# syl051088/DynaAlign

Hardware: AMD Instinct MI355X
Metric: sequence-pairs/sec (MinHash k=4 n_hash=500; NW BLOSUM62) at 1/2/4/8 MI355X (higher is better)
Workload: dtype u32

## Files before the change

dynaalign_amd/csrc/api.cpp:

```cpp
#include <sched.h>

#include <algorithm>
#include <atomic>
#include <chrono>
#include <climits>
#include <cmath>
#include <condition_variable>
#include <cstddef>
#include <map>
#include <memory>
#include <cstdlib>
#include <cstring>
#include <functional>
#include <mutex>
#include <random>
#include <string>
#include <thread>
#include <vector>

#include "da_common.hpp"

namespace da { size_t destroy_cached_comms(); }

namespace da {
// ... 345 lines not shown
  c.mh_no_pipe = env_flag("DYNAALIGN_MH_NO_PIPE");
  c.mh_pipe_one_stream = env_flag("DYNAALIGN_MH_PIPE_ONE_STREAM");
  c.mh_dedup_min_n = env_i64("DYNAALIGN_MH_DEDUP_MIN_N", -1);
  c.mh_dedup_max_pct = env_i64("DYNAALIGN_MH_DEDUP_MAX_PCT", -1);
  c.mh_sparse_max_pairs = std::min<uint64_t>(env_u64("DYNAALIGN_MH_SPARSE_MAX_PAIRS", 400000000ull), 0xfffffff0ull);
  c.mh_no_hybrid = env_flag("DYNAALIGN_MH_NO_HYBRID");
  c.mh_hybrid_min_n = env_i64("DYNAALIGN_MH_HYBRID_MIN_N", -1);
  c.mh_hybrid_dedup = env_flag("DYNAALIGN_MH_HYBRID_DEDUP");
  if (const char *e = getenv("DYNAALIGN_MH_EXPAND"))
    c.mh_expand = !strcmp(e, "rows") ? MH_EXPAND_ROWS : !strcmp(e, "rowspipe") ? MH_EXPAND_ROWSPIPE : !strcmp(e, "pipe") ? MH_EXPAND_PIPE
                : !strcmp(e, "tiles") ? MH_EXPAND_TILES : MH_EXPAND_DEFAULT;
  c.mh_pipe_step = (int)std::max<int64_t>(0, env_i64("DYNAALIGN_MH_PIPE_STEP", 0));
  c.mh_pipe_wg = (int)std::max<int64_t>(0, std::min<int64_t>(4, env_i64("DYNAALIGN_MH_PIPE_WG", 0)));
  c.mh_pipe_head = (int)std::max<int64_t>(0, env_i64("DYNAALIGN_MH_PIPE_HEAD", 0));
  c.mh_expand_zones = (int)env_i64("DYNAALIGN_MH_EXPAND_ZONES", 0);
  const int pb = (int)env_i64("DYNAALIGN_PLANE_BITS", 0);
  c.plane_bits = (pb == 32 || pb == 16 || pb == 15 || pb == 14 || pb == 12) ? pb : 0;
  c.k2_no_asm = env_flag("DYNAALIGN_K2_NO_ASM");
  c.k2_persist = env_flag("DYNAALIGN_K2_PERSIST");
  c.k2_wg_per_cu = (int)std::max<int64_t>(0, env_i64("DYNAALIGN_K2_WG_PER_CU", 0));
  c.nw_no_dedup = env_flag("DYNAALIGN_NW_NO_DEDUP");
  c.nw_int32 = env_flag("DYNAALIGN_NW_INT32");
  c.nw_no_prefix = env_flag("DYNAALIGN_NW_NO_PREFIX_SHARE");
  c.nw_dedup_min_n = env_i64("DYNAALIGN_NW_DEDUP_MIN_N", -1);
  c.no_host_widen = env_flag("DYNAALIGN_NO_HOST_WIDEN");
  c.plain_d2h = env_flag("DYNAALIGN_PLAIN_D2H");
  c.no_buffer_cache = env_flag("DYNAALIGN_NO_BUFFER_CACHE");
  c.d2h_threads = (int)std::max<int64_t>(0, env_i64("DYNAALIGN_D2H_THREADS", 0));
  c.buffer_cache_pct = (int)std::max<int64_t>(0, std::min<int64_t>(90, env_i64("DYNAALIGN_BUFFER_CACHE_PCT", 30)));
  c.block_bytes = env_u64("DYNAALIGN_BLOCK_BYTES", 0);
// ... 200 lines not shown
    (void)hipStreamSynchronize(r->side); (void)hipStreamSynchronize(r->alt[0]); (void)hipStreamSynchronize(r->alt[1]);
    std::lock_guard<std::mutex> g(pipe_pool().m);
    pipe_pool().idle[r->dev & 63].push_back(r);
  }
};
static int count_unique(const uint8_t *d_bytes, const int64_t *d_offsets, int64_t n, const NwDedupPlan &p, hipStream_t stream, int64_t *U) {
  int rc;
  if ((rc = launch_nw_dedup_count(d_bytes, d_offsets, n, p, stream)) != DA_OK) return rc;
  int32_t M = 0, S = 0;
  DA_HIP_TRY(hipMemcpyAsync(&M, p.pm + n, 4, hipMemcpyDeviceToHost, stream));
  DA_HIP_TRY(hipMemcpyAsync(&S, p.ps + n, 4, hipMemcpyDeviceToHost, stream));
  DA_HIP_TRY(hipStreamSynchronize(stream));
  *U = (int64_t)M + S; return DA_OK;
}
enum MhForm { MH_DIRECT = 0, MH_TILES = 1, MH_SPARSE = 2, MH_TILES_PIPE = 3, MH_ROWS = 4, MH_ROWS_PIPE = 5 };
struct MhRoute { int64_t n = 0, unique = 0, hybrid_pairs = -1; int taken = MH_DIRECT, plane_bits = 0, chunks = 0, expand_launches = 0, hybrid_bits_before = 0; bool packed_table = false; float ms[6] = {0, 0, 0, 0, 0, 0}; };
static MhRoute &mh_route() { static thread_local MhRoute r; return r; }
struct MhEvents {
  hipEvent_t e[7] = {nullptr, nullptr, nullptr, nullptr, nullptr, nullptr, nullptr};
  ~MhEvents() { for (hipEvent_t x : e) if (x) (void)hipEventDestroy(x); }
  hipEvent_t operator[](int i) const { return e[i]; }
  static void ms(MhRoute &r, int i, hipEvent_t from, hipEvent_t to) { (void)hipEventElapsedTime(&r.ms[i], from, to); }
  void steps(MhRoute &r, int count) const { for (int i = 0; i < count; ++i) ms(r, i, e[i], e[i + 1]); }
};
struct LaunchUnion {
  hipEvent_t origin; float total = 0, covered_to = 0;
  void add(hipEvent_t begin, hipEvent_t end) {
    float b = 0, e = 0;
    (void)hipEventElapsedTime(&b, origin, begin); (void)hipEventElapsedTime(&e, origin, end);
    if (e > covered_to) { total += e - std::max(b, covered_to); covered_to = e; }
  }
};
struct MhDedup { int64_t U = 0; bool take = false, rows = false; DevBuf work; NwDedupPlan p{}; std::vector<int32_t> ub; };
static int mh_count_unique(const uint8_t *d_res, const int64_t *d_off, int64_t n, int64_t total, DevBuf *work, NwDedupPlan *p, int64_t *U,
                           hipStream_t stream) {
  int rc;
  if ((rc = work->alloc(nw_dedup_workspace_bytes(n, total))) != DA_OK) return rc;
  *p = nw_dedup_layout(work->p, n, total);
  return count_unique(d_res, d_off, n, *p, stream, U);
}
static int mh_dedup_plan(const uint8_t *d_res, const int64_t *d_off, int64_t n, int64_t total, int n_hash, const double *d_out, int64_t ld,
                         MhDedup *d, hipStream_t stream) {
  const Config &cfg = da::config();
  int rc;
  d->U = n;
  const int64_t min_n = cfg.mh_dedup_min_n >= 0 ? cfg.mh_dedup_min_n : 2048;
  if (n < min_n || n > 0x7ffffff0LL || total <= 0 || n_hash > 2047 || cfg.mh_no_dedup) return DA_OK;
  if ((rc = mh_count_unique(d_res, d_off, n, total, &d->work, &d->p, &d->U, stream)) != DA_OK) return rc;
  const int64_t U = d->U;
  const int64_t max_pct = cfg.mh_dedup_max_pct >= 0 ? cfg.mh_dedup_max_pct
                        : expand_stream_ok(n, std::min<int64_t>(U, 65536), n_hash, d_out, ld) ? 68 : 60;
  d->take = U > 0 && U * 100 <= n * max_pct && expand_rows_workspace_bytes(n, U, DA_OUT_F64, false, n_hash, 0) != 0;
  if (!d->take) return DA_OK;
  if ((rc = launch_nw_dedup_build(d_res, d_off, n, U, d->p, stream, true)) != DA_OK) return rc;
  d->rows = cfg.mh_expand <= MH_EXPAND_ROWSPIPE && expand_stream_ok(n, U, n_hash, d_out, ld);
  if (d->rows) return DA_OK;
  const int64_t NB = mh_sym_bands(n);
  std::vector<int32_t> b((size_t)NB);
  d->ub.resize((size_t)NB + 1);
  DA_HIP_TRY(hipMemcpy2DAsync(d->ub.data(), 4, d->p.pm, 4096, 4, (size_t)NB, hipMemcpyDeviceToHost, stream));
  DA_HIP_TRY(hipMemcpy2DAsync(b.data(), 4, d->p.ps, 4096, 4, (size_t)NB, hipMemcpyDeviceToHost, stream));
  DA_HIP_TRY(hipStreamSynchronize(stream));
  for (int64_t q = 0; q < NB; ++q) d->ub[(size_t)q] += b[(size_t)q];
  d->ub[(size_t)NB] = (int32_t)U;
  return DA_OK;
}
constexpr int HY_KEEP = 254;
enum class MhOperand { dense, sparse, split };
struct MhAdmission { MhOperand form = MhOperand::dense; uint64_t pairs = 0; const uint16_t *codes = nullptr, *dense = nullptr; int64_t ld_ids = 0; };
static int mh_admit(const Dictionary &dict, void *d_work, int64_t n, int n_hash, bool ask_sparse, int split_from_bits, MhAdmission *a,
// ... 226 lines not shown
}
}

static int mh_full_symmetric(const uint8_t *d_res, const int64_t *d_off, int64_t n, int64_t total, int k, int n_hash,
                             const uint32_t *d_seeds, double *d_out, int64_t ld, hipStream_t stream) {
  const Config &cfg = da::config();
  int rc;
  MhRoute &route = mh_route() = MhRoute();
  route.n = n;
  MhEvents ev;
  for (auto &e : ev.e) DA_HIP_TRY(hipEventCreate(&e));
  DA_HIP_TRY(hipEventRecord(ev[0], stream));
  MhDedup d;
  if ((rc = mh_dedup_plan(d_res, d_off, n, total, n_hash, d_out, ld, &d, stream)) != DA_OK) return rc;
  route.unique = d.U;
  DA_HIP_TRY(hipEventRecord(ev[1], stream));
  MhCodes c;
  if ((rc = mh_codes(d.take ? d.p.ucodes : d_res, d.take ? d.p.uoff : d_off, d.take ? d.U : n, k, n_hash, d_seeds, !d.take && d.U * 10 >= n * 9,
                     d.take && !cfg.mh_hybrid_dedup ? 13 : 12, &c, stream)) != DA_OK) return rc;
  route.plane_bits = c.bits;
  if (c.split()) { route.hybrid_pairs = (int64_t)c.adm.pairs; route.hybrid_bits_before = c.dict.bits_data; }
  DA_HIP_TRY(hipEventRecord(ev[2], stream));
  MhCall call{n, n_hash, d_out, ld, stream, route, ev, c, d};
  if (!d.take) return c.adm.form == MhOperand::sparse ? mh_sparse(call) : mh_direct(call);
  DevBuf dtab, ex;
  call.pk = d.rows && !c.split() && mh_compare_pk_ok(d.U, n_hash, c.bits);
  route.packed_table = call.pk;
  call.ld_d = call.pk ? pk_lo_bytes(d.U) : (d.U + 7) / 8 * 8;
  if ((rc = dtab.alloc(call.pk ? pk_table_bytes(d.U) : (size_t)d.U * (size_t)call.ld_d * 2)) != DA_OK) return rc;
  if ((rc = ex.alloc(d.rows ? expand_stream_scratch_bytes(n, d.U) : expand_rows_workspace_bytes(n, d.U, DA_OUT_F64, false, n_hash, 0))) != DA_OK) return rc;
// ... 13 lines not shown
  if (n_hash > 65535) return fail(DA_ERR_UNSUPPORTED, "the compare kernel counts in 16 bits: n_hash <= 65535 (got %d); da_similarity_mh handles more", n_hash);
  return mh_full_symmetric(d_residues, d_offsets, n, total_residues, k, n_hash, d_seeds, d_out, ld, static_cast<hipStream_t>(stream));
}

int da_mh_last_route_chunks(int *chunks_out, int *expand_launches_out) {
  const MhRoute &r = mh_route();
  if (chunks_out) *chunks_out = r.chunks;
  if (expand_launches_out) *expand_launches_out = r.expand_launches;
  return DA_OK;
}

int da_mh_last_route_split(int64_t *rare_incidences_out, int *plane_bits_without_out) {
  const MhRoute &r = mh_route();
  if (rare_incidences_out) *rare_incidences_out = r.hybrid_pairs;
  if (plane_bits_without_out) *plane_bits_without_out = r.hybrid_bits_before;
  return DA_OK;
}

extern "C" int da_debug_mh_last_table_packed(int *packed_out) {
  if (!packed_out) return fail(DA_ERR_BAD_ARG, "NULL pointer");
  *packed_out = mh_route().packed_table ? 1 : 0;
  return DA_OK;
}

int da_mh_last_route(int64_t *n_out, int64_t *unique_out, int *dedup_taken_out, int *plane_bits_out, double *ms6_out) {
  const MhRoute &r = mh_route();
  if (n_out) *n_out = r.n;
  if (unique_out) *unique_out = r.unique;
  if (dedup_taken_out) *dedup_taken_out = r.taken;
  if (plane_bits_out) *plane_bits_out = r.plane_bits;
// ... 68 lines not shown
  MhCrossRoute &route = mh_cross_route() = MhCrossRoute();
  route.m = m; route.n = n; route.ux = m; route.uy = n;
  CrossEvents ev;
  for (auto &e : ev.e) DA_HIP_TRY(hipEventCreate(&e));
  DA_HIP_TRY(hipEventRecord(ev.e[0], stream));
  CrossSide sx, sy;
  bool take = false;
  const int64_t min_n = cfg.mh_dedup_min_n >= 0 ? cfg.mh_dedup_min_n : 2048;
  if (!cfg.mh_no_dedup && m + n >= min_n && x_total > 0 && y_total > 0 && n_hash <= 2047) {
    if ((rc = mh_count_unique(d_x_residues, d_x_offsets, m, x_total, &sx.work, &sx.p, &sx.U, stream)) != DA_OK ||
        (rc = mh_count_unique(d_y_residues, d_y_offsets, n, y_total, &sy.work, &sy.p, &sy.U, stream)) != DA_OK) return rc;
    route.ux = sx.U; route.uy = sy.U;
    const double pct = (double)(cfg.mh_dedup_max_pct >= 0 ? cfg.mh_dedup_max_pct : 68);
    take = sx.U > 0 && sy.U > 0 && (double)sx.U * (double)sy.U * 10000.0 <= (double)m * (double)n * pct * pct &&
           expand_stream_rect_ok(m, n, sx.U, sy.U, n_hash, d_out, ld);
    if (take && ((rc = launch_nw_dedup_build(d_x_residues, d_x_offsets, m, sx.U, sx.p, stream, true)) != DA_OK ||
                 (rc = launch_nw_dedup_build(d_y_residues, d_y_offsets, n, sy.U, sy.p, stream, true)) != DA_OK)) return rc;
  }
  DA_HIP_TRY(hipEventRecord(ev.e[1], stream));
  MhCrossOperand c;
  if ((rc = take ? mh_cross_operand(sx.p.ucodes, sx.p.uoff, sx.U, sy.p.ucodes, sy.p.uoff, sy.U, k, n_hash, d_seeds, &c, stream)
                 : mh_cross_operand(d_x_residues, d_x_offsets, m, d_y_residues, d_y_offsets, n, k, n_hash, d_seeds, &c, stream)) != DA_OK) return rc;
  route.plane_bits = c.bits;
  DA_HIP_TRY(hipEventRecord(ev.e[2], stream));
  DevBuf dtab, ex;
  if (!take) {
    if ((rc = mh_cross_compare(c, n_hash, 0, m, DA_OUT_F64, d_out, ld, stream)) != DA_OK) return rc;
    DA_HIP_TRY(hipEventRecord(ev.e[3], stream));
  } else {
    const int64_t ld_d = (sy.U + 7) / 8 * 8;
    if ((rc = dtab.alloc((size_t)sx.U * (size_t)ld_d * 2)) != DA_OK || (rc = ex.alloc(expand_stream_scratch_bytes(m, sx.U))) != DA_OK) return rc;
    if ((rc = mh_cross_compare(c, n_hash, 0, sx.U, DA_OUT_COMPACT, dtab.p, ld_d, stream)) != DA_OK) return rc;
// ... 2925 lines not shown
```

dynaalign_amd/csrc/da_common.hpp:

```cpp
#pragma once

#include <hip/hip_runtime.h>

#include <cstdarg>
#include <cstdint>
#include <cstdio>
#include <string>

#include "../../include/dynaalign.h"

namespace da {
struct Config {
  bool mh_no_dedup = false, mh_no_sparse = false, mh_no_pipe = false, mh_pipe_one_stream = false;
  int64_t mh_dedup_min_n = -1, mh_dedup_max_pct = -1;
  uint64_t mh_sparse_max_pairs = 400000000ull;
  bool mh_no_hybrid = false, mh_hybrid_dedup = false;
  int64_t mh_hybrid_min_n = -1;
  int mh_expand = 0;
  int mh_pipe_step = 0, mh_pipe_wg = 0, mh_pipe_head = 0;
  int mh_expand_zones = 0;
  int plane_bits = 0;
  bool k2_no_asm = false, k2_persist = false;
  int k2_wg_per_cu = 0;
  bool nw_no_dedup = false, nw_int32 = false, nw_no_prefix = false;
  int64_t nw_dedup_min_n = -1;
  bool no_host_widen = false, plain_d2h = false, no_buffer_cache = false;
  int d2h_threads = 0, buffer_cache_pct = 30;
  uint64_t block_bytes = 0;
  bool trace = false, louvain_debug = false;
  int louvain_threads = 0;
};
const Config &config();


std::string &last_error_ref();
// ... 61 lines not shown
__host__ __device__ inline int64_t pad16_base_words(int64_t n, int n_hash) { return 2 * plane_geom(n, n_hash, 16).copy_words; }
__host__ __device__ inline int64_t pad16_slot_word(int64_t n, int n_hash, int64_t row, int group) {
  const int64_t nst = (n_hash + 31) / 32;
  return (((row >> 7) * nst + group) * 128 + k2_slot((int)(row & 127))) * K2_PAD16_SLOT_WORDS;
}
inline int64_t mh_planes_words(int64_t n, int n_hash) {
  if (n <= 0 || n_hash <= 0) return 0;
  const int64_t raw = 2 * plane_geom(n, n_hash, 32).copy_words;
  const int64_t p16 = pad16_base_words(n, n_hash) + 2 * pad16_copy_words(n, n_hash);
  return raw > p16 ? raw : p16;
}

__host__ __device__ inline int64_t pk_lo_bytes(int64_t U) { return (U + 127) / 128 * 128; }
__host__ __device__ inline int64_t pk_row_bytes(int64_t lo_bytes) { return lo_bytes + lo_bytes / 8; }
inline size_t pk_table_bytes(int64_t U) { return (size_t)U * (size_t)pk_row_bytes(pk_lo_bytes(U)); }

int launch_minhash_signatures(const uint8_t *d_res, const int64_t *d_off, int64_t n,
                              int k, int n_hash, const uint32_t *d_seeds, uint32_t *d_sig,
                              int64_t ld_sig, hipStream_t stream);
int launch_mh_compare(const uint32_t *d_planes, int64_t n, int n_hash,
                      int64_t row_begin, int64_t row_end, bool symmetric, int kind,
                      void *d_out, int64_t ld, hipStream_t stream, int plane_bits = 32, int tile_stride = 1,
                      bool upper_only = false, int fold_q = 0, int64_t fold_w = 0);
int launch_mh_compare_rect(const uint32_t *d_planes, int64_t n, int n_hash, int64_t row_begin, int64_t row_end, int64_t col_begin, int64_t col_end,
                           int kind, void *d_out, int64_t ld, hipStream_t stream, int plane_bits);
int launch_fill_sig_rows(uint32_t *d_sig, int64_t ld_sig, int64_t m, int64_t m_pad, int n_hash, hipStream_t stream);
int64_t mh_sym_bands(int64_t n);
int64_t mh_sym_band_prefix(int64_t n, int64_t band);
bool mh_compare_bands_ok(int64_t n, int n_hash, int plane_bits, const void *d_out, int64_t ld);
int launch_mh_compare_bands_u16(const uint32_t *d_planes, int64_t n, int n_hash, uint16_t *d_out, int64_t ld, int64_t band_begin,
// ... 47 lines not shown
                   nullptr, nullptr, nullptr, c0, c1);
}
size_t nw_sort_unique_workspace_bytes(int64_t n);
int launch_nw_sort_unique(const uint8_t *d_codes, const int64_t *d_off, int64_t n, void *d_work, size_t work_bytes, const int32_t **perm_out,
                          const uint8_t **lcp_out, hipStream_t stream);
struct NwDedupPlan {
  uint32_t *table; uint32_t table_size;
  int32_t *rep, *mult, *last, *fm, *fs, *pm, *ps, *uid_of, *uidx, *ufirst, *ulast, *ulen, *minfirst, *maxlast;
  int64_t *uoff;
  uint8_t *ucodes;
  size_t bytes;
};
NwDedupPlan nw_dedup_layout(void *work, int64_t n, int64_t total);
size_t nw_dedup_workspace_bytes(int64_t n, int64_t total);
int launch_nw_dedup_count(const uint8_t *d_codes, const int64_t *d_off, int64_t n, const NwDedupPlan &p, hipStream_t stream);
int launch_nw_dedup_build(const uint8_t *d_codes, const int64_t *d_off, int64_t n, int64_t U, const NwDedupPlan &p, hipStream_t stream,
                          bool first_order = false);
int launch_expand_unique(const uint16_t *d_D, int64_t ld_d, const int32_t *d_uidx, int64_t n, int kind, bool is_nw, int n_hash,
                         void *d_out, int64_t ld, hipStream_t stream, int nw_max_len = 0, uint16_t *d_F = nullptr,
                         const int32_t *d_ufirst = nullptr, int64_t U = 0, hipEvent_t after_gather = nullptr, hipEvent_t after_rows = nullptr,
                         int table_world = 1, int64_t table_rows_local = 0,
                         bool only_leftover = false);
bool expand_stream_ok(int64_t n, int64_t U, int n_hash, const void *d_out, int64_t ld);
size_t expand_stream_scratch_bytes(int64_t n, int64_t U);
bool expand_stream_packed(int n_hash);
int launch_expand_stream(const uint16_t *d_D, int64_t ld_d, const int32_t *d_uidx, int64_t n, int64_t U, int n_hash, double *d_out, int64_t ld,
                         void *d_scratch, hipStream_t stream, hipEvent_t after_lists = nullptr, bool pk = false);
int launch_expand_stream_lists(const int32_t *d_uidx, int64_t n, int64_t U, void *d_scratch, hipStream_t stream);
bool expand_stream_rect_ok(int64_t m, int64_t n, int64_t U_x, int64_t U_y, int n_hash, const void *d_out, int64_t ld);
int launch_expand_stream_rect(const uint16_t *d_D, int64_t ld_d, const int32_t *d_uidx_x, int64_t m, int64_t U_x, const int32_t *d_uidx_y, int64_t n,
                              int64_t U_y, int n_hash, double *d_out, int64_t ld, void *d_scratch, hipStream_t stream,
                              hipEvent_t after_lists = nullptr);
int launch_expand_stream_rows(const uint16_t *d_D, int64_t ld_d, const int32_t *d_uidx, int64_t n, int64_t U, int n_hash, double *d_out, int64_t ld,
                              void *d_scratch, int64_t row_end, hipStream_t stream,
                              bool pk = false);
int launch_expand_rows(const uint16_t *d_F, int64_t ld_f, const int32_t *d_uidx, int64_t n, bool is_nw, int n_hash, int nw_max_len,
                       double *d_out, int64_t ld, int64_t band_begin, int64_t band_end, hipStream_t stream);
size_t expand_rows_workspace_bytes(int64_t n, int64_t U, int kind, bool is_nw, int n_hash, int nw_max_len);
int launch_upper_histogram(const uint16_t *d_m, int64_t ld, int64_t n, int nbins, unsigned long long *d_hist,
                           hipStream_t stream, int rank = 0, int world = 0, const int32_t *d_rowmap = nullptr);
// ... 69 lines not shown
```

dynaalign_amd/csrc/minhash_kernels.hip:

```cpp
#include "da_common.hpp"

#include <algorithm>
#include <atomic>
#include <mutex>
#include <vector>
#include <type_traits>

namespace da {
namespace {

__device__ __forceinline__ uint32_t rotl32(uint32_t v, int r) {
  return __builtin_rotateleft32(v, r);
}
__device__ __forceinline__ uint32_t mm3_scramble(uint32_t w) {
  w *= 0xcc9e2d51u;
  w = rotl32(w, 15);
  w *= 0x1b873593u;
  return w;
}
__device__ __forceinline__ uint32_t mm3_mix(uint32_t h, uint32_t kk) {
  h ^= kk;
  return rotl32(h, 13) * 5u + 0xe6546b64u;
}
__device__ __forceinline__ uint32_t mm3_final(uint32_t h, uint32_t len) {
// ... 1638 lines not shown
    }
  } else {
    for (int e = tid; e < tab_entries; e += 256) tab[e] = (double)e / (double)n_hash;
  }
#pragma unroll
  for (int q = 0; q < 8; ++q)
    *reinterpret_cast<uint4 *>(er_lds + ((tid >> 4) + 16 * q) * ER_STRIDE + (tid & 15) * 16) = st[q];
  __syncthreads();
  auto widen = [&](uint32_t x) -> double {
    if (IS_NW) return tab[(x >> 8) * (uint32_t)tab_stride + (x & 255u)];
    return tab[x];
  };
  er_store_tile(er_lds, widen, out, ld, I0, J0, tx, ty);
}

constexpr int ES_THREADS = 1024, ES_COPIES = 4, ES_ZONES = 8, ES_BATCH = 16;
__global__ __launch_bounds__(256) void k_es_zero(uint32_t *__restrict__ w, int words) {
  const int i = blockIdx.x * 256 + threadIdx.x;
  if (i < words) w[i] = 0u;
}
__global__ __launch_bounds__(256) void k_es_count(const int32_t *__restrict__ uidx, int n, int U, int Z, uint32_t *__restrict__ cnt) {
  const int i = blockIdx.x * 256 + threadIdx.x;
  if (i < n) atomicAdd(&cnt[(i / Z) * U + uidx[i]], 1u);
}
__device__ __forceinline__ uint64_t es_scan_load(const uint32_t *__restrict__ cnt, int K, int i) {
  const uint32_t c = i < K ? cnt[i] : 0u;
  return (uint64_t)c | ((uint64_t)((c + ES_COPIES - 1) / ES_COPIES) << 32);
}
__global__ __launch_bounds__(1024) void k_es_scan_sums(const uint32_t *__restrict__ cnt, int K, uint64_t *__restrict__ bsum) {
  __shared__ uint64_t wsum[16];
  uint64_t x = es_scan_load(cnt, K, blockIdx.x * 1024 + threadIdx.x);
// ... 61 lines not shown
  if (i < K) {
    const uint32_t first = zstart[i], cnt = zstart[i + 1] - first;
    for (uint32_t q = 0; q < cnt; ++q) items[first + q] = make_int2(i % U, (int)(q * ES_COPIES));
  }
}
__device__ __forceinline__ double es_ratio(uint32_t c, double dn, double rcp) {
  const double dc = (double)c, q0 = __dmul_rn(dc, rcp), e = __fma_rn(-q0, dn, dc);
  return __fma_rn(e, rcp, q0);
}
__global__ __launch_bounds__(256) void k_es_ratio_check(int n_hash, double *__restrict__ out) {
  const int c = blockIdx.x * 256 + threadIdx.x;
  const double dn = (double)n_hash, rcp = 1.0 / dn;
  if (c <= n_hash) out[c] = es_ratio((uint32_t)c, dn, rcp);
}
enum { ES_U16 = 0, ES_U16_PK = 1, ES_PK = 2 };
template <int FMT, int NQ>
__global__ __launch_bounds__(ES_THREADS, 8)
void k_expand_stream(const uint16_t *__restrict__ D, int64_t ld_d, const int32_t *__restrict__ uidx,
                                                              const uint32_t *__restrict__ cstart, const int32_t *__restrict__ cpos,
                                                              const int2 *__restrict__ items, const uint32_t *__restrict__ zstart, int U, int zones,
                                                              int row_end, int n, int n_hash, double *__restrict__ out, int64_t ld,
                                                              uint32_t *ticket, int max_batch) {
  extern __shared__ __attribute__((aligned(16))) unsigned char es_lds[];
#ifdef ES_PRIO
  __builtin_amdgcn_s_setprio(ES_PRIO);
#endif
  constexpr bool PACKED = FMT != ES_U16;
  uint16_t *row = reinterpret_cast<uint16_t *>(es_lds);
  unsigned char *row_lo = es_lds, *row_hi = row_lo + ld_d;
  const int tid = threadIdx.x;
// ... 18 lines not shown
  asm volatile("s_getreg_b32 %0, hwreg(HW_REG_XCC_ID)" : "=s"(home));
  home = (home & 7u) % (unsigned)zones;
  const uint32_t home_z0 = zstart[home * U], home_lim = zstart[home * U + row_end] - home_z0,
                 home_all = zstart[home * U + U] - home_z0;
  const uint32_t share = max(1u, gridDim.x / (unsigned)zones);
  auto take = [&]() {
    int tz = -1, tk = 0, te = 0;
    for (int t = 0; t < zones && tz < 0; ++t) {
      const int z = (int)((home + (unsigned)t) % (unsigned)zones);
      const uint32_t z0 = t ? zstart[z * U] : home_z0, lim = t ? zstart[z * U + row_end] - z0 : home_lim,
                     all = t ? zstart[z * U + U] - z0 : home_all;
      uint32_t cur = __hip_atomic_load(&ticket[z], __ATOMIC_RELAXED, __HIP_MEMORY_SCOPE_AGENT);
      while (cur < lim) {
        const uint32_t b = min(min((uint32_t)max_batch, lim - cur), max(1u, (all - cur) / share));
        const uint32_t old = atomicCAS(&ticket[z], cur, cur + b);
        if (old == cur) { tz = z; tk = (int)(z0 + cur); te = tk + (int)b; break; }
        cur = old;
      }
    }
    s_zone = tz; s_next = tk; s_end = te;
  };
  if (tid == 0) take();
  __syncthreads();
  int z = __builtin_amdgcn_readfirstlane(s_zone), k = __builtin_amdgcn_readfirstlane(s_next), k_end = __builtin_amdgcn_readfirstlane(s_end);
  int2 it = z >= 0 ? items[k] : make_int2(0, 0);
  if (z >= 0) ES_FETCH(it.x)
  const int2 *u2 = reinterpret_cast<const int2 *>(uidx);
  const int j2_end = n >> 1;
  while (z >= 0) {
    __syncthreads();
// ... 42 lines not shown
    k = kn;
  }
#undef ES_FETCH
}

bool expand_stream_ok(int64_t n, int64_t U, int n_hash, const void *d_out, int64_t ld) {
  return n >= 2 && n <= 0x7fffffffLL && U >= 1 && U <= 65536 && n_hash >= 1 && n_hash <= 2047 && (ld & 1) == 0 &&
         (reinterpret_cast<uintptr_t>(d_out) & 15) == 0;
}
extern "C" int da_debug_ratio_check(int n_hash, double *d_out, void *stream) {
  if (n_hash < 1 || !d_out) return fail(DA_ERR_BAD_ARG, "ratio check: bad arguments");
  hipLaunchKernelGGL(k_es_ratio_check, dim3((unsigned)(n_hash / 256 + 1)), dim3(256), 0, static_cast<hipStream_t>(stream), n_hash, d_out);
  DA_HIP_TRY(hipGetLastError());
  return DA_OK;
}
bool expand_stream_packed(int n_hash) { return n_hash <= 511; }
static int es_zones() { return config().mh_expand_zones == 1 ? 1 : ES_ZONES; }
struct EsLists { uint32_t *cnt, *cursor, *ticket, *cstart, *zstart; int32_t *cpos; int2 *items; uint64_t *bsum; int zones, Z, K; size_t bytes; };
static EsLists es_layout(void *d_scratch, int64_t n, int64_t U, int zones) {
  uint32_t *w = static_cast<uint32_t *>(d_scratch);
  EsLists L;
  const int64_t K = (int64_t)zones * U;
  L.zones = zones; L.Z = (int)ceil_div(n, zones); L.K = (int)K;
  L.cnt = w; L.cursor = w + K; L.ticket = w + 2 * K; L.cstart = L.ticket + ES_ZONES; L.zstart = L.cstart + (K + 1);
  L.cpos = reinterpret_cast<int32_t *>(L.zstart + (K + 1));
  L.items = reinterpret_cast<int2 *>((reinterpret_cast<uintptr_t>(L.cpos + n) + 15) & ~(uintptr_t)15);
  L.bsum = reinterpret_cast<uint64_t *>(L.items + (std::min(n, K) + n / ES_COPIES + 2));
  L.bytes = (size_t)(reinterpret_cast<unsigned char *>(L.bsum + (ceil_div(K, 1024) + 1)) - static_cast<unsigned char *>(d_scratch));
  return L;
}
size_t expand_stream_scratch_bytes(int64_t n, int64_t U) {
  return es_layout(nullptr, n, U, ES_ZONES).bytes + 16;
}
static int es_lists(const int32_t *d_uidx, int64_t n, int64_t U, void *d_scratch, int zones, hipStream_t stream) {
  const EsLists L = es_layout(d_scratch, n, U, zones);
  const int zero_words = 2 * L.K + ES_ZONES;
  hipLaunchKernelGGL(k_es_zero, dim3((unsigned)ceil_div(zero_words, 256)), dim3(256), 0, stream, L.cnt, zero_words);
  const unsigned nblk = (unsigned)ceil_div(L.K, 1024);
// ... 737 lines not shown
```

dynaalign_amd/csrc/nw_kernels.hip:

```cpp
#include <algorithm>
#include <climits>
#include <cstdlib>

#include <hipcub/hipcub.hpp>

#include "da_common.hpp"

namespace da {
namespace {

#include "blosum_data.inc"

struct ScoreTable { signed char s[576]; };

__device__ __forceinline__ int aa_index(uint32_t c) {
  switch (c) {
    case 'A': return 0;  case 'R': return 1;  case 'N': return 2;  case 'D': return 3;
    case 'C': return 4;  case 'Q': return 5;  case 'E': return 6;  case 'G': return 7;
    case 'H': return 8;  case 'I': return 9;  case 'L': return 10; case 'K': return 11;
    case 'M': return 12; case 'F': return 13; case 'P': return 14; case 'S': return 15;
    case 'T': return 16; case 'W': return 17; case 'Y': return 18; case 'V': return 19;
    case 'B': return 20; case 'Z': return 21; case 'X': return 22; case '*': return 23;
    default: return -1;
  }
// ... 641 lines not shown
  const uint64_t e = woff + x - v;
  if (i < n) {
    if (MODE == 0) { o0[i] = (int32_t)(uint32_t)e; o1[i] = (int32_t)(uint32_t)(e >> 32); }
    else o64[i] = (int64_t)e;
  }
  if (blockIdx.x == gridDim.x - 1 && tid == 0) {
    const uint64_t t = bsum[gridDim.x];
    if (MODE == 0) { o0[n] = (int32_t)(uint32_t)t; o1[n] = (int32_t)(uint32_t)(t >> 32); }
    else o64[n] = (int64_t)t;
  }
}
__global__ __launch_bounds__(256) void k_dd_assign(const int32_t *__restrict__ rep, const int32_t *__restrict__ mult,
                                                   const int32_t *__restrict__ last, const int32_t *__restrict__ pm,
                                                   const int32_t *__restrict__ ps, const int64_t *__restrict__ off, int32_t n,
                                                   int32_t *__restrict__ uid_of, int32_t *__restrict__ ufirst,
                                                   int32_t *__restrict__ ulast, int32_t *__restrict__ ulen, int first_order) {
  const int32_t i = blockIdx.x * 256 + threadIdx.x;
  if (i >= n || rep[i] != i) return;
  const int32_t M = pm[n];
  const int32_t uid = first_order ? pm[i] + ps[i] : (mult[i] > 1 ? pm[i] : M + ps[i]);
  uid_of[i] = uid;
  ufirst[uid] = i;
  ulast[uid] = last[i];
  ulen[uid] = (int32_t)(off[i + 1] - off[i]);
}
__global__ __launch_bounds__(256) void k_dd_map(const int32_t *__restrict__ rep, const int32_t *__restrict__ uid_of, int32_t n,
                                                int32_t *__restrict__ uidx) {
  const int32_t i = blockIdx.x * 256 + threadIdx.x;
  if (i < n) uidx[i] = uid_of[rep[i]];
}
__global__ __launch_bounds__(256) void k_dd_gather(const uint8_t *__restrict__ codes, const int64_t *__restrict__ off,
                                                   const int32_t *__restrict__ ufirst, const int64_t *__restrict__ uoff, int32_t U,
                                                   uint8_t *__restrict__ ucodes) {
  const int32_t u = blockIdx.x * 256 + threadIdx.x;
  if (u >= U) return;
// ... 45 lines not shown
  hipLaunchKernelGGL(k_dd_lookup, dim3(nb), dim3(256), 0, stream, d_codes, d_off, (int32_t)n, p.table, p.table_size - 1, p.rep, p.mult, p.last);
  hipLaunchKernelGGL(k_dd_flags, dim3(nb), dim3(256), 0, stream, p.rep, p.mult, (int32_t)n, p.fm, p.fs);
  const bool wide_scan = true;
  if (n >= 8192 && wide_scan) {
    const int32_t nblk = (int32_t)ceil_div(n, 1024);
    uint64_t *bsum = reinterpret_cast<uint64_t *>(p.table);
    hipLaunchKernelGGL(k_dd_scan_sums<0>, dim3((unsigned)nblk), dim3(1024), 0, stream, p.fm, p.fs, (int32_t)n, bsum);
    hipLaunchKernelGGL(k_dd_scan_offsets, dim3(1), dim3(1024), 0, stream, bsum, nblk);
    hipLaunchKernelGGL(k_dd_scan_apply<0>, dim3((unsigned)nblk), dim3(1024), 0, stream, p.fm, p.fs, (int32_t)n, bsum, p.pm, p.ps, (int64_t *)nullptr);
  } else
    hipLaunchKernelGGL(k_dd_scan_pair, dim3(1), dim3(1024), 0, stream, p.fm, p.fs, p.pm, p.ps, (int32_t)n);
  DA_HIP_TRY(hipGetLastError());
  return DA_OK;
}
int launch_nw_dedup_build(const uint8_t *d_codes, const int64_t *d_off, int64_t n, int64_t U, const NwDedupPlan &p, hipStream_t stream,
                          bool first_order) {
  const unsigned nb = (unsigned)ceil_div(n, 256);
  hipLaunchKernelGGL(k_dd_assign, dim3(nb), dim3(256), 0, stream, p.rep, p.mult, p.last, p.pm, p.ps, d_off, (int32_t)n, p.uid_of,
                     p.ufirst, p.ulast, p.ulen, first_order ? 1 : 0);
  hipLaunchKernelGGL(k_dd_map, dim3(nb), dim3(256), 0, stream, p.rep, p.uid_of, (int32_t)n, p.uidx);
  if (U >= 8192) {
    const int32_t nblk = (int32_t)ceil_div(U, 1024);
    uint64_t *bsum = reinterpret_cast<uint64_t *>(p.table);
    hipLaunchKernelGGL(k_dd_scan_sums<1>, dim3((unsigned)nblk), dim3(1024), 0, stream, p.ulen, (const int32_t *)nullptr, (int32_t)U, bsum);
    hipLaunchKernelGGL(k_dd_scan_offsets, dim3(1), dim3(1024), 0, stream, bsum, nblk);
    hipLaunchKernelGGL(k_dd_scan_apply<1>, dim3((unsigned)nblk), dim3(1024), 0, stream, p.ulen, (const int32_t *)nullptr, (int32_t)U, bsum, (int32_t *)nullptr,
                       (int32_t *)nullptr, p.uoff);
  } else
    hipLaunchKernelGGL(k_dd_scan<int64_t>, dim3(1), dim3(1024), 0, stream, p.ulen, p.uoff, (int32_t)U);
  hipLaunchKernelGGL(k_dd_gather, dim3((unsigned)ceil_div(U, 256)), dim3(256), 0, stream, d_codes, d_off, p.ufirst, p.uoff, (int32_t)U, p.ucodes);
  hipLaunchKernelGGL(k_dd_blocks, dim3((unsigned)ceil_div(U, 64)), dim3(64), 0, stream, p.ufirst, p.ulast, (int32_t)U, p.minfirst, p.maxlast);
  DA_HIP_TRY(hipGetLastError());
  return DA_OK;
}
// ... 245 lines not shown
```

Before: 329.2 billion.

## Assign zone-interleaved unique IDs for singletons on the MinHash rows dedup path

Adds a 'zoned' dedup ordering: multi-occurrence uniques keep low IDs, and singleton uniques are ranked by interleaving across the row zones used by the stream expander, rather than in plain first-seen order. It becomes the default when the rows/stream expansion path is taken. The apparent goal is to balance per-zone work and improve ticket-stealing locality in k_expand_stream. It also adds debug entry points and an optional steal counter compiled in only under ES_STEAL_COUNT. The cost is a small shared-memory histogram and a rank computation per unique in k_dd_assign.

```diff
diff --git a/dynaalign_amd/csrc/api.cpp b/dynaalign_amd/csrc/api.cpp
--- a/dynaalign_amd/csrc/api.cpp
+++ b/dynaalign_amd/csrc/api.cpp
@@ -383,6 +383,7 @@
   c.mh_pipe_wg = (int)std::max<int64_t>(0, std::min<int64_t>(4, env_i64("DYNAALIGN_MH_PIPE_WG", 0)));
   c.mh_pipe_head = (int)std::max<int64_t>(0, env_i64("DYNAALIGN_MH_PIPE_HEAD", 0));
   c.mh_expand_zones = (int)env_i64("DYNAALIGN_MH_EXPAND_ZONES", 0);
+  if (const char *e = getenv("DYNAALIGN_MH_DEDUP_ORDER")) c.mh_dedup_order = !strcmp(e, "first") ? 1 : !strcmp(e, "zoned") ? 2 : 0;
   const int pb = (int)env_i64("DYNAALIGN_PLANE_BITS", 0);
   c.plane_bits = (pb == 32 || pb == 16 || pb == 15 || pb == 14 || pb == 12) ? pb : 0;
   c.k2_no_asm = env_flag("DYNAALIGN_K2_NO_ASM");
@@ -613,7 +614,7 @@
   *U = (int64_t)M + S; return DA_OK;
 }
 enum MhForm { MH_DIRECT = 0, MH_TILES = 1, MH_SPARSE = 2, MH_TILES_PIPE = 3, MH_ROWS = 4, MH_ROWS_PIPE = 5 };
-struct MhRoute { int64_t n = 0, unique = 0, hybrid_pairs = -1; int taken = MH_DIRECT, plane_bits = 0, chunks = 0, expand_launches = 0, hybrid_bits_before = 0; bool packed_table = false; float ms[6] = {0, 0, 0, 0, 0, 0}; };
+struct MhRoute { int64_t n = 0, unique = 0, hybrid_pairs = -1; int taken = MH_DIRECT, plane_bits = 0, chunks = 0, expand_launches = 0, hybrid_bits_before = 0, dedup_order = -1; bool packed_table = false; float ms[6] = {0, 0, 0, 0, 0, 0}; };
 static MhRoute &mh_route() { static thread_local MhRoute r; return r; }
 struct MhEvents {
   hipEvent_t e[7] = {nullptr, nullptr, nullptr, nullptr, nullptr, nullptr, nullptr};
@@ -630,7 +631,7 @@
     if (e > covered_to) { total += e - std::max(b, covered_to); covered_to = e; }
   }
 };
-struct MhDedup { int64_t U = 0; bool take = false, rows = false; DevBuf work; NwDedupPlan p{}; std::vector<int32_t> ub; };
+struct MhDedup { int64_t U = 0; bool take = false, rows = false; DedupOrder order = DedupOrder::first; DevBuf work; NwDedupPlan p{}; std::vector<int32_t> ub; };
 static int mh_count_unique(const uint8_t *d_res, const int64_t *d_off, int64_t n, int64_t total, DevBuf *work, NwDedupPlan *p, int64_t *U,
                            hipStream_t stream) {
   int rc;
@@ -651,8 +652,9 @@
                         : expand_stream_ok(n, std::min<int64_t>(U, 65536), n_hash, d_out, ld) ? 68 : 60;
   d->take = U > 0 && U * 100 <= n * max_pct && expand_rows_workspace_bytes(n, U, DA_OUT_F64, false, n_hash, 0) != 0;
   if (!d->take) return DA_OK;
-  if ((rc = launch_nw_dedup_build(d_res, d_off, n, U, d->p, stream, true)) != DA_OK) return rc;
   d->rows = cfg.mh_expand <= MH_EXPAND_ROWSPIPE && expand_stream_ok(n, U, n_hash, d_out, ld);
+  d->order = d->rows && cfg.mh_dedup_order != 1 ? DedupOrder::zoned : DedupOrder::first;
+  if ((rc = launch_nw_dedup_build(d_res, d_off, n, U, d->p, stream, d->order, d->rows ? expand_stream_zones() : 1)) != DA_OK) return rc;
   if (d->rows) return DA_OK;
   const int64_t NB = mh_sym_bands(n);
   std::vector<int32_t> b((size_t)NB);
@@ -909,6 +911,7 @@
   MhDedup d;
   if ((rc = mh_dedup_plan(d_res, d_off, n, total, n_hash, d_out, ld, &d, stream)) != DA_OK) return rc;
   route.unique = d.U;
+  if (d.take) route.dedup_order = (int)d.order;
   DA_HIP_TRY(hipEventRecord(ev[1], stream));
   MhCodes c;
   if ((rc = mh_codes(d.take ? d.p.ucodes : d_res, d.take ? d.p.uoff : d_off, d.take ? d.U : n, k, n_hash, d_seeds, !d.take && d.U * 10 >= n * 9,
@@ -952,6 +955,38 @@
   const MhRoute &r = mh_route();
   if (rare_incidences_out) *rare_incidences_out = r.hybrid_pairs;
   if (plane_bits_without_out) *plane_bits_without_out = r.hybrid_bits_before;
+  return DA_OK;
+}
+
+extern "C" int da_debug_mh_last_dedup_order(int *order_out) {
+  if (!order_out) return fail(DA_ERR_BAD_ARG, "NULL pointer");
+  *order_out = mh_route().dedup_order;
+  return DA_OK;
+}
+extern "C" int da_debug_mh_dedup_ids(const uint8_t *d_res, const int64_t *d_off, int64_t n, int64_t total, int order, int zones, int32_t *d_uidx_out,
+                                     int64_t *unique_out, int64_t *multi_out, void *stream) {
+  if (zones == 0) zones = expand_stream_zones();
+  if (!d_res || !d_off || !d_uidx_out || n < 1 || n > 0x7ffffff0LL || total <= 0 || order < 0 || order > 2 || zones < 1 || zones > ES_ZONES)
+    return fail(DA_ERR_BAD_ARG, "dedup ids: bad arguments");
+  const hipStream_t st = static_cast<hipStream_t>(stream);
+  DevBuf work;
+  NwDedupPlan p{};
+  int64_t U = 0;
+  int32_t M = 0;
+  int rc;
+  if ((rc = mh_count_unique(d_res, d_off, n, total, &work, &p, &U, st)) != DA_OK) return rc;
+  if ((rc = launch_nw_dedup_build(d_res, d_off, n, U, p, st, static_cast<DedupOrder>(order), zones)) != DA_OK) return rc;
+  DA_HIP_TRY(hipMemcpyAsync(d_uidx_out, p.uidx, (size_t)n * 4, hipMemcpyDeviceToDevice, st));
+  DA_HIP_TRY(hipMemcpyAsync(&M, p.pm + n, 4, hipMemcpyDeviceToHost, st));
+  DA_HIP_TRY(hipStreamSynchronize(st));
+  if (unique_out) *unique_out = U;
+  if (multi_out) *multi_out = M;
+  return DA_OK;
+}
+extern "C" int da_debug_zoned_ids(const int32_t *h, int zones, int64_t M, int64_t *ids_out) {
+  if (!h || !ids_out || zones < 1 || zones > ES_ZONES || M < 0) return fail(DA_ERR_BAD_ARG, "zoned ids: bad arguments");
+  for (int z = 0; z < zones; ++z)
+    for (int64_t q = 0; q < h[z]; ++q) *ids_out++ = M + zoned_rank(h, zones, z, q);
   return DA_OK;
 }
 
@@ -1050,8 +1085,8 @@
     const double pct = (double)(cfg.mh_dedup_max_pct >= 0 ? cfg.mh_dedup_max_pct : 68);
     take = sx.U > 0 && sy.U > 0 && (double)sx.U * (double)sy.U * 10000.0 <= (double)m * (double)n * pct * pct &&
            expand_stream_rect_ok(m, n, sx.U, sy.U, n_hash, d_out, ld);
-    if (take && ((rc = launch_nw_dedup_build(d_x_residues, d_x_offsets, m, sx.U, sx.p, stream, true)) != DA_OK ||
-                 (rc = launch_nw_dedup_build(d_y_residues, d_y_offsets, n, sy.U, sy.p, stream, true)) != DA_OK)) return rc;
+    if (take && ((rc = launch_nw_dedup_build(d_x_residues, d_x_offsets, m, sx.U, sx.p, stream, DedupOrder::first)) != DA_OK ||
+                 (rc = launch_nw_dedup_build(d_y_residues, d_y_offsets, n, sy.U, sy.p, stream, DedupOrder::first)) != DA_OK)) return rc;
   }
   DA_HIP_TRY(hipEventRecord(ev.e[1], stream));
   MhCrossOperand c;
diff --git a/dynaalign_amd/csrc/da_common.hpp b/dynaalign_amd/csrc/da_common.hpp
--- a/dynaalign_amd/csrc/da_common.hpp
+++ b/dynaalign_amd/csrc/da_common.hpp
@@ -19,6 +19,7 @@
   int mh_expand = 0;
   int mh_pipe_step = 0, mh_pipe_wg = 0, mh_pipe_head = 0;
   int mh_expand_zones = 0;
+  int mh_dedup_order = 0;
   int plane_bits = 0;
   bool k2_no_asm = false, k2_persist = false;
   int k2_wg_per_cu = 0;
@@ -110,6 +111,14 @@
 __host__ __device__ inline int64_t pk_lo_bytes(int64_t U) { return (U + 127) / 128 * 128; }
 __host__ __device__ inline int64_t pk_row_bytes(int64_t lo_bytes) { return lo_bytes + lo_bytes / 8; }
 inline size_t pk_table_bytes(int64_t U) { return (size_t)U * (size_t)pk_row_bytes(pk_lo_bytes(U)); }
+
+constexpr int ES_ZONES = 8;
+__host__ __device__ inline int64_t zone_rows(int64_t n, int zones) { return (n + zones - 1) / zones; }
+__host__ __device__ inline int64_t zoned_rank(const int32_t *h, int zones, int z, int64_t q) {
+  int64_t r = 0;
+  for (int t = 0; t < zones; ++t) r += ((int64_t)h[t] < q ? (int64_t)h[t] : q) + ((t < z && (int64_t)h[t] > q) ? 1 : 0);
+  return r;
+}
 
 int launch_minhash_signatures(const uint8_t *d_res, const int64_t *d_off, int64_t n,
                               int k, int n_hash, const uint32_t *d_seeds, uint32_t *d_sig,
@@ -187,8 +196,9 @@
 NwDedupPlan nw_dedup_layout(void *work, int64_t n, int64_t total);
 size_t nw_dedup_workspace_bytes(int64_t n, int64_t total);
 int launch_nw_dedup_count(const uint8_t *d_codes, const int64_t *d_off, int64_t n, const NwDedupPlan &p, hipStream_t stream);
+enum class DedupOrder { multi_first = 0, first = 1, zoned = 2 };
 int launch_nw_dedup_build(const uint8_t *d_codes, const int64_t *d_off, int64_t n, int64_t U, const NwDedupPlan &p, hipStream_t stream,
-                          bool first_order = false);
+                          DedupOrder order = DedupOrder::multi_first, int zones = 1);
 int launch_expand_unique(const uint16_t *d_D, int64_t ld_d, const int32_t *d_uidx, int64_t n, int kind, bool is_nw, int n_hash,
                          void *d_out, int64_t ld, hipStream_t stream, int nw_max_len = 0, uint16_t *d_F = nullptr,
                          const int32_t *d_ufirst = nullptr, int64_t U = 0, hipEvent_t after_gather = nullptr, hipEvent_t after_rows = nullptr,
@@ -197,6 +207,7 @@
 bool expand_stream_ok(int64_t n, int64_t U, int n_hash, const void *d_out, int64_t ld);
 size_t expand_stream_scratch_bytes(int64_t n, int64_t U);
 bool expand_stream_packed(int n_hash);
+int expand_stream_zones();
 int launch_expand_stream(const uint16_t *d_D, int64_t ld_d, const int32_t *d_uidx, int64_t n, int64_t U, int n_hash, double *d_out, int64_t ld,
                          void *d_scratch, hipStream_t stream, hipEvent_t after_lists = nullptr, bool pk = false);
 int launch_expand_stream_lists(const int32_t *d_uidx, int64_t n, int64_t U, void *d_scratch, hipStream_t stream);
diff --git a/dynaalign_amd/csrc/minhash_kernels.hip b/dynaalign_amd/csrc/minhash_kernels.hip
--- a/dynaalign_amd/csrc/minhash_kernels.hip
+++ b/dynaalign_amd/csrc/minhash_kernels.hip
@@ -1676,7 +1676,7 @@
   er_store_tile(er_lds, widen, out, ld, I0, J0, tx, ty);
 }
 
-constexpr int ES_THREADS = 1024, ES_COPIES = 4, ES_ZONES = 8, ES_BATCH = 16;
+constexpr int ES_THREADS = 1024, ES_COPIES = 4, ES_BATCH = 16;
 __global__ __launch_bounds__(256) void k_es_zero(uint32_t *__restrict__ w, int words) {
   const int i = blockIdx.x * 256 + threadIdx.x;
   if (i < words) w[i] = 0u;
@@ -1768,6 +1768,9 @@
   if (c <= n_hash) out[c] = es_ratio((uint32_t)c, dn, rcp);
 }
 enum { ES_U16 = 0, ES_U16_PK = 1, ES_PK = 2 };
+#ifdef ES_STEAL_COUNT
+__device__ unsigned es_steal[64][ES_ZONES][2];
+#endif
 template <int FMT, int NQ>
 __global__ __launch_bounds__(ES_THREADS, 8)
 void k_expand_stream(const uint16_t *__restrict__ D, int64_t ld_d, const int32_t *__restrict__ uidx,
@@ -1816,6 +1819,9 @@
       while (cur < lim) {
         const uint32_t b = min(min((uint32_t)max_batch, lim - cur), max(1u, (all - cur) / share));
         const uint32_t old = atomicCAS(&ticket[z], cur, cur + b);
+#ifdef ES_STEAL_COUNT
+        if (old == cur) atomicAdd(&es_steal[min(63, (row_end + 1023) >> 10)][home][t ? 1 : 0], b);
+#endif
         if (old == cur) { tz = z; tk = (int)(z0 + cur); te = tk + (int)b; break; }
         cur = old;
       }
@@ -1888,14 +1894,24 @@
   DA_HIP_TRY(hipGetLastError());
   return DA_OK;
 }
+#ifdef ES_STEAL_COUNT
+extern "C" int da_debug_expand_steals(unsigned *out, int reset) {
+  static const unsigned zero[64 * ES_ZONES * 2] = {};
+  DA_HIP_TRY(hipDeviceSynchronize());
+  if (out) DA_HIP_TRY(hipMemcpyFromSymbol(out, HIP_SYMBOL(es_steal), sizeof(zero)));
+  if (reset) DA_HIP_TRY(hipMemcpyToSymbol(HIP_SYMBOL(es_steal), zero, sizeof(zero)));
+  return DA_OK;
+}
+#endif
 bool expand_stream_packed(int n_hash) { return n_hash <= 511; }
 static int es_zones() { return config().mh_expand_zones == 1 ? 1 : ES_ZONES; }
+int expand_stream_zones() { return es_zones(); }
 struct EsLists { uint32_t *cnt, *cursor, *ticket, *cstart, *zstart; int32_t *cpos; int2 *items; uint64_t *bsum; int zones, Z, K; size_t bytes; };
 static EsLists es_layout(void *d_scratch, int64_t n, int64_t U, int zones) {
   uint32_t *w = static_cast<uint32_t *>(d_scratch);
   EsLists L;
   const int64_t K = (int64_t)zones * U;
-  L.zones = zones; L.Z = (int)ceil_div(n, zones); L.K = (int)K;
+  L.zones = zones; L.Z = (int)zone_rows(n, zones); L.K = (int)K;
   L.cnt = w; L.cursor = w + K; L.ticket = w + 2 * K; L.cstart = L.ticket + ES_ZONES; L.zstart = L.cstart + (K + 1);
   L.cpos = reinterpret_cast<int32_t *>(L.zstart + (K + 1));
   L.items = reinterpret_cast<int2 *>((reinterpret_cast<uintptr_t>(L.cpos + n) + 15) & ~(uintptr_t)15);
diff --git a/dynaalign_amd/csrc/nw_kernels.hip b/dynaalign_amd/csrc/nw_kernels.hip
--- a/dynaalign_amd/csrc/nw_kernels.hip
+++ b/dynaalign_amd/csrc/nw_kernels.hip
@@ -679,11 +679,25 @@
                                                    const int32_t *__restrict__ last, const int32_t *__restrict__ pm,
                                                    const int32_t *__restrict__ ps, const int64_t *__restrict__ off, int32_t n,
                                                    int32_t *__restrict__ uid_of, int32_t *__restrict__ ufirst,
-                                                   int32_t *__restrict__ ulast, int32_t *__restrict__ ulen, int first_order) {
+                                                   int32_t *__restrict__ ulast, int32_t *__restrict__ ulen, int order, int zones, int32_t Z) {
+  __shared__ int32_t h[ES_ZONES];
+  if (order == (int)DedupOrder::zoned) {
+    if ((int)threadIdx.x < zones) {
+      const int64_t lo = min((int64_t)n, (int64_t)threadIdx.x * Z), hi = min((int64_t)n, ((int64_t)threadIdx.x + 1) * Z);
+      h[threadIdx.x] = ps[hi] - ps[lo];
+    }
+    __syncthreads();
+  }
   const int32_t i = blockIdx.x * 256 + threadIdx.x;
   if (i >= n || rep[i] != i) return;
   const int32_t M = pm[n];
-  const int32_t uid = first_order ? pm[i] + ps[i] : (mult[i] > 1 ? pm[i] : M + ps[i]);
+  int32_t uid;
+  if (order == (int)DedupOrder::first) uid = pm[i] + ps[i];
+  else if (mult[i] > 1) uid = pm[i];
+  else if (order == (int)DedupOrder::zoned) {
+    const int32_t z = i / Z;
+    uid = M + (int32_t)zoned_rank(h, zones, z, (int64_t)(ps[i] - ps[(int64_t)z * Z]));
+  } else uid = M + ps[i];
   uid_of[i] = uid;
   ufirst[uid] = i;
   ulast[uid] = last[i];
@@ -759,10 +773,11 @@
   return DA_OK;
 }
 int launch_nw_dedup_build(const uint8_t *d_codes, const int64_t *d_off, int64_t n, int64_t U, const NwDedupPlan &p, hipStream_t stream,
-                          bool first_order) {
+                          DedupOrder order, int zones) {
+  if (zones < 1 || zones > ES_ZONES) return fail(DA_ERR_BAD_ARG, "dedupe plan: zones must be 1 ... %d (got %d)", ES_ZONES, zones);
   const unsigned nb = (unsigned)ceil_div(n, 256);
   hipLaunchKernelGGL(k_dd_assign, dim3(nb), dim3(256), 0, stream, p.rep, p.mult, p.last, p.pm, p.ps, d_off, (int32_t)n, p.uid_of,
-                     p.ufirst, p.ulast, p.ulen, first_order ? 1 : 0);
+                     p.ufirst, p.ulast, p.ulen, (int)order, zones, (int32_t)zone_rows(n, zones));
   hipLaunchKernelGGL(k_dd_map, dim3(nb), dim3(256), 0, stream, p.rep, p.uid_of, (int32_t)n, p.uidx);
   if (U >= 8192) {
     const int32_t nblk = (int32_t)ceil_div(U, 1024);
```

Measured after the change: 351.0 billion (median of 6 runs). 6.6% higher.
